# ZJU-FAST-Lab/Dftpav

Measured on AMD Instinct MI355X. Metric: trajectory solves/sec (batched), 16-piece MINCO, higher is better.
Workload: dtype f64

## Files before the change

dftpav_amd/csrc/capi.cpp:

```cpp
#include <hip/hip_runtime.h>
#include <dlfcn.h>
#include <atomic>
#include <mutex>

#include <climits>
#include <cmath>
#include <cstdio>
#include <algorithm>
#include <cstdlib>
#include <cstring>
#include <string>
#include <vector>

#include "../../include/dftpav_hip.h"
#include "device_types.h"
#include "e4_plan.h"
#include "traj_math.h"
#include "cr_trig.h"
#include "rs_math.h"
#include "search_args.h"
#include "plan_args.h"

namespace dftpav {
hipError_t launch_solver(const DevBatch &D, const DevBatch *d_dev, int mode, int threads, int grid, SchedArgs sched,
// ... 79 lines not shown
  void *d_search_ws = nullptr;
  size_t search_ws_bytes = 0;
};

struct dftpav_batch {
  dftpav_handle *h = nullptr;
  int B = 0;
  int n_active = 0;
  DevLayout L{};
  DevParams P{};
  int threads = 0;
  bool op_in_lds = false, cor_in_lds = false;
  bool have_corridor = false;
  bool sched = false;
  int slots = 0, slice = 0, hand_over = 0;
  int threads2 = 0;
  bool op_in_lds2 = false, cor_in_lds2 = false;
  int *d_queue = nullptr, *d_stragglers = nullptr, *d_stragglers2 = nullptr, *d_sflag = nullptr, *d_iota = nullptr;
  int qcap = 0;
  bool pending = false;
  unsigned *d_qctl = nullptr;
  double *d_state = nullptr;
  DevBatch *d_dev2 = nullptr;
  E4Sizes e4{}, e4b{};
  int *d_e4[2][5] = {{nullptr, nullptr, nullptr, nullptr, nullptr}, {nullptr, nullptr, nullptr, nullptr, nullptr}};
  int NptsPad = 0;
  std::vector<double> x0_host;
  bool uploaded = false;
  double t_now = 0.0, epis = 0.0;
  double *d_x0 = nullptr, *d_iniS = nullptr, *d_finS = nullptr, *d_corridor = nullptr;
  int16_t *d_pt_piece = nullptr, *d_pt_j = nullptr;
  double *d_opM[kMaxSeg] = {nullptr}, *d_opMT[kMaxSeg] = {nullptr};
  double *d_histS = nullptr, *d_histY = nullptr, *d_histU = nullptr, *d_histV = nullptr, *d_histR = nullptr;
  double *d_x_in = nullptr, *d_x_out = nullptr, *d_f = nullptr, *d_g = nullptr;
  int *d_status = nullptr, *d_success = nullptr, *d_iters = nullptr, *d_evals = nullptr;
  long long *d_hist = nullptr, *d_ticks = nullptr, *d_prof = nullptr;
  unsigned char *d_records = nullptr;
  unsigned char *h_records = nullptr;
  DevBatch *d_dev = nullptr;
  int dev_version = -1;
  DevBatch *h_stage = nullptr;
  hipEvent_t stage_ev = nullptr;
  bool stage_busy = false;
  bool prof_on = false;
  double *d_coef = nullptr, *d_dt = nullptr;
  double *d_f_eval = nullptr;
  double *d_trace = nullptr;
  double *d_cor_raw = nullptr;
  int order = DFTPAV_ORDER_DEVICE;
  int ref_S = 0;
  double *d_ref_tab = nullptr, *d_ref_scratch = nullptr;
  RefPlan ref_plan{};
  double *d_cor_t = nullptr;
  bool cor_t_dirty = true;
  bool cor_rect = false, cor_t_rect = false;
  int *d_rect_flag = nullptr;
  bool coef_override = false;
  int residency = -1;
  struct PlanCycle {
    double *d_poses = nullptr, *d_t = nullptr, *d_v = nullptr, *d_rd = nullptr;
    int *d_col = nullptr, *d_first = nullptr, *d_valid = nullptr;
    size_t n_poses = 0, n_t = 0, n_v = 0, n_rd = 0;
    std::vector<double> poses, tt, vv;
    int n_samples = 0;
    bool in_flight = false;
  } pc;
// ... 864 lines not shown
  P.surround_clearance = p.surround_clearance;
  P.max_vel[0] = p.max_forward_vel; P.max_vel[1] = p.max_backward_vel;
  P.max_acc[0] = p.max_forward_acc; P.max_acc[1] = p.max_backward_acc;
  P.max_cur[0] = p.max_forward_cur; P.max_cur[1] = p.max_backward_cur;
  P.non_sinv = p.non_sinv;
  P.mini_T = p.mini_T;
  P.fail_cost = p.fail_cost;
  double W = p.veh_width + 2 * p.half_margin, Lh = p.veh_length + 2 * p.half_margin, dcr = p.veh_d_cr;
  P.veh_length_infl = Lh;
  double le[4][2] = {{dcr + Lh / 2.0, W / 2.0}, {dcr + Lh / 2.0, -W / 2.0}, {dcr - Lh / 2.0, -W / 2.0},
                     {dcr - Lh / 2.0, W / 2.0}};
  for (int k = 0; k < 4; k++) { P.vec_le[k][0] = le[k][0]; P.vec_le[k][1] = le[k][1]; }
  P.vec_le[4][0] = le[0][0]; P.vec_le[4][1] = le[0][1];
  fill_footprint_edges(P);
  P.gear_opt = p.gear_opt;
  P.mem_size = p.lbfgs_mem_size;
  P.past = p.lbfgs_past;
  P.max_iterations = p.lbfgs_max_iterations;
  P.max_linesearch = p.lbfgs_max_linesearch;
  P.delta = p.lbfgs_delta;
  P.g_epsilon = p.lbfgs_g_epsilon;
  P.min_step = p.lbfgs_min_step;
  P.max_step = p.lbfgs_max_step;
  P.f_dec_coeff = p.lbfgs_f_dec_coeff;
  P.s_curv_coeff = p.lbfgs_s_curv_coeff;
  P.cautious_factor = p.lbfgs_cautious_factor;
  P.machine_prec = p.lbfgs_machine_prec;
}

extern "C" void dftpav_batch_destroy(dftpav_batch *b) {
  if (!b) return;
  (void)hipSetDevice(b->h->device);
  (void)hipStreamSynchronize(b->h->stream);
  void *ptrs[] = {b->d_x0, b->d_iniS, b->d_finS, b->d_corridor, b->d_pt_piece, b->d_pt_j, b->d_histS, b->d_histU, b->d_histV, b->d_histR,
                  b->d_x_in, b->d_x_out, b->d_f, b->d_g, b->d_status, b->d_success, b->d_iters, b->d_evals,
                  b->d_hist, b->d_ticks, b->d_prof, b->d_dev, b->d_coef, b->d_dt, b->d_records,
                  b->d_queue, b->d_stragglers, b->d_stragglers2, b->d_sflag, b->d_iota, b->d_qctl, b->d_state, b->d_dev2,
                  b->d_f_eval, b->d_trace, b->d_cor_raw, b->d_ref_tab, b->d_ref_scratch, b->d_cor_t, b->d_rect_flag, b->pc.d_poses, b->pc.d_t, b->pc.d_v, b->pc.d_rd, b->pc.d_col, b->pc.d_first,
                  b->pc.d_valid};
  {
    auto &v = b->h->batches;
    v.erase(std::remove(v.begin(), v.end(), b), v.end());
  }
  for (void *p : ptrs)
    if (p) (void)hipFree(p);
  if (b->h_records) (void)hipHostFree(b->h_records);
  for (int w = 0; w < 2; w++)
    for (int t = 0; t < 5; t++)
      if (b->d_e4[w][t]) (void)hipFree(b->d_e4[w][t]);
  for (int i = 0; i < kMaxSeg; i++) {
    if (b->d_opM[i]) (void)hipFree(b->d_opM[i]);
    if (b->d_opMT[i]) (void)hipFree(b->d_opMT[i]);
  }
  if (b->h_stage) (void)hipHostFree(b->h_stage);
  if (b->stage_ev) (void)hipEventDestroy(b->stage_ev);
  if (b->ev0) (void)hipEventDestroy(b->ev0);
  if (b->ev1) (void)hipEventDestroy(b->ev1);
  delete b;
}

static void fill_dev_layout(const dftpav_layout &layout, int K, int Kd, DevLayout &L) {
  L = DevLayout{};
  L.M = layout.M;
  L.H = layout.H;
  L.K = K;
  L.Kd = Kd;
  L.Kmax = L.K > L.Kd ? L.K : L.Kd;
// ... 398 lines not shown
  D.e4_groups = b->e4.groups;
  D.e4_left = b->e4.left;
  D.e4_lcap = b->e4.lcap;
  D.e4_gtab = b->d_e4[0][0];
  D.e4_ltab = b->d_e4[0][1];
  D.e4_wave = b->d_e4[0][2];
  D.e4_round = b->d_e4[0][3];
  D.e4_piece = b->d_e4[0][4];
  int off = 0;
  for (int i = 0; i < kMaxSeg; i++) {
    D.opM[i] = b->d_opM[i];
    D.opMT[i] = b->d_opMT[i];
    D.op_off[i] = off;
    if (i < b->L.M) off += 6 * b->L.piece_nums[i] * (b->L.piece_nums[i] + 5);
  }
  dftpav_handle *h = b->h;
  D.sur.S = h->S;
  D.sur_np = h->sur_pieces;
  D.sur_coef_lds = sur_coef_in_lds(b, b->threads, b->op_in_lds, b->cor_in_lds);
  D.sur.piece_off = h->d_sur_off;
  D.sur.durations = h->d_sur_dur;
  D.sur.theta = h->d_sur_theta;
  D.sur.bbox = h->d_sur_bbox;
  D.sur.coeffs = h->d_sur_coef;
  D.sur.total = h->d_sur_total;
  D.sur.start = h->d_sur_start;
  D.t_now = b->t_now;
  D.epis = b->epis;
  D.histS = b->d_histS;
  D.histY = b->d_histY;
  D.histU = b->d_histU;
  D.histV = b->d_histV;
  D.histR = b->d_histR;
  D.queue = b->d_queue;
  D.qctl = b->d_qctl;
  D.stragglers = b->d_stragglers;
  D.stragglers2 = b->d_stragglers2;
  D.qcap = b->qcap;
  D.state = b->d_state;
  D.sflag = b->d_sflag;
  D.state_stride = solver_state_doubles(b->L, b->P);
  D.x_in = b->d_x_in;
  D.x_out = b->d_x_out;
  D.f_out = b->d_f;
  D.g_out = b->d_g;
  D.f_eval = b->d_f_eval;
  D.status = b->d_status;
  D.success = b->d_success;
  D.iters = b->d_iters;
  D.evals = b->d_evals;
  D.hist_sum = b->d_hist;
  D.ticks = b->d_ticks;
  D.records = b->d_records;
  D.records_host = b->h_records;
  D.prof = b->prof_on ? b->d_prof : nullptr;
  D.coef_out = b->d_coef;
  D.dt_out = b->d_dt;
  D.trace = b->d_trace;
  D.trace_b = b->trace_b;
  D.trace_cap = b->trace_cap;
  D.trace_n = b->trace_n;
  return D;
}

static int sync_dev(dftpav_batch *b, DevBatch &D) {
  dftpav_handle *h = b->h;
// ... 257 lines not shown
  if (order == DFTPAV_ORDER_REFERENCE && b->d_trace) {
    h->err = "reference order: dftpav_batch_trace is a device-order facility -- switch the trace off first";
    return DFTPAV_E_UNSUPPORTED;
  }
  HIPCHK(h, hipSetDevice(h->device));
  if (int rc = finish_pending(b)) return rc;
  HIPCHK(h, hipStreamSynchronize(h->stream));
  if (order == DFTPAV_ORDER_REFERENCE) {
    if (!reference_order_supported(b->L, b->P, h->S)) {
      h->err = "reference order: n <= 256 variables, H <= 12 half-planes, 5 H + S + 4 <= 64 terms per point, every gear segment >= 2 pieces, 159 KB of LDS";
      return DFTPAV_E_UNSUPPORTED;
    }
    int n_cu = 256;
    hipDeviceProp_t prop;
    if (hipGetDeviceProperties(&prop, h->device) == hipSuccess && prop.multiProcessorCount > 0) n_cu = prop.multiProcessorCount;
    const RefPlan pl = reference_order_plan(b->L, b->P, h->S, b->B, n_cu, b->residency == 2, ref_options_from_env());
    if (pl.kind != kRefTeam && ensure_ring_buffers(b) != hipSuccess) {
      h->err = "reference order: no device memory for the ring of this batch";
      return DFTPAV_E_HIP;
    }
    const bool new_tab = !b->d_ref_tab || !b->d_ref_scratch || b->ref_S != h->S;
    std::vector<double> tab;
    for (int sg = 0; new_tab && sg < b->L.M; sg++) {
      std::vector<double> one;
      if (!reference_order_tables(b->L.piece_nums[sg], one)) {
        h->err = "reference order: the LU factors of this band system do not have the pattern the kernel assumes";
        return DFTPAV_E_UNSUPPORTED;
      }
      std::vector<double> packed(reference_order_table_doubles(b->L.piece_nums[sg]));
      reference_order_pack_tables(b->L.piece_nums[sg], one.data(), packed.data());
      tab.insert(tab.end(), packed.begin(), packed.end());
    }
    double *cor_t = b->d_cor_t, *d_tab = nullptr, *d_scr = nullptr;
    auto undo = [&](const char *msg) {
      if (cor_t != b->d_cor_t) (void)hipFree(cor_t);
      if (d_tab) (void)hipFree(d_tab);
      if (d_scr) (void)hipFree(d_scr);
      (void)hipGetLastError();
      h->err = msg;
      return DFTPAV_E_HIP;
    };
    if (pl.kind >= kRefQuad && !cor_t && hipMalloc(&cor_t, sizeof(double) * reference_order_quad_corridor_doubles(b->L, b->B)) != hipSuccess)
      return undo("reference order: no device memory for the QUAD shape's copy of the corridor");
    if (new_tab && (hipMalloc(&d_tab, sizeof(double) * tab.size()) != hipSuccess ||
                    hipMalloc(&d_scr, sizeof(double) * reference_order_scratch_doubles(b->L, b->B, h->S)) != hipSuccess ||
                    hipMemcpy(d_tab, tab.data(), sizeof(double) * tab.size(), hipMemcpyHostToDevice) != hipSuccess))
      return undo("reference order: no device memory for the term records of this batch");
    if (new_tab) {
      if (b->d_ref_tab) (void)hipFree(b->d_ref_tab);
      if (b->d_ref_scratch) (void)hipFree(b->d_ref_scratch);
      b->d_ref_tab = d_tab;
      b->d_ref_scratch = d_scr;
      b->ref_S = h->S;
    }
    if (pl.kind >= kRefQuad) b->cor_t_dirty = true;
    b->d_cor_t = cor_t;
    b->ref_plan = pl;
  }
  b->order = order;
  b->solved = false;
  return DFTPAV_OK;
}
extern "C" int dftpav_batch_get_order(const dftpav_batch *b) { return b ? b->order : DFTPAV_E_INVALID; }

extern "C" int dftpav_batch_eval(dftpav_batch *b, const double *x, double *f, double *g) {
  if (!b || !x || !b->uploaded || !b->have_corridor) return DFTPAV_E_INVALID;
  dftpav_handle *h = b->h;
  const size_t nb = (size_t)b->B * b->L.n;
  HIPCHK(h, hipSetDevice(h->device));
  HIPCHK(h, hipMemcpyAsync(b->d_x_in, x, sizeof(double) * nb, hipMemcpyHostToDevice, h->stream));
  DevBatch D;
  if (int rc = sync_dev(b, D)) return rc;
  HIPCHK(h, launch_for(b, D, kModeEval));
  if (f) HIPCHK(h, hipMemcpyAsync(f, b->d_f_eval, sizeof(double) * b->B, hipMemcpyDeviceToHost, h->stream));
  if (g) HIPCHK(h, hipMemcpyAsync(g, b->d_g, sizeof(double) * nb, hipMemcpyDeviceToHost, h->stream));
  HIPCHK(h, hipStreamSynchronize(h->stream));
  return DFTPAV_OK;
}

static int launch_stragglers(dftpav_batch *b, const DevBatch &D, int source) {
  dftpav_handle *h = b->h;
  DevBatch D2 = D;
  D2.op_in_lds = b->op_in_lds2 ? 1 : 0;
  D2.cor_in_lds = b->cor_in_lds2 ? 1 : 0;
  D2.sur_coef_lds = sur_coef_in_lds(b, b->threads2, b->op_in_lds2, b->cor_in_lds2);
  D2.e4_rounds = b->e4b.rounds;
  D2.e4_groups = b->e4b.groups;
  D2.e4_left = b->e4b.left;
  D2.e4_lcap = b->e4b.lcap;
// ... 1715 lines not shown
```

dftpav_amd/csrc/device_types.h:

```cpp
#pragma once
#include <cstdint>

#ifndef DFTPAV_HD
#if defined(__HIPCC__)
#define DFTPAV_HD __host__ __device__
#else
#define DFTPAV_HD
#endif
#endif

namespace dftpav {

constexpr int kMaxSeg = 8;
constexpr int kWave = 64;
constexpr int kMaxThreads = 1024;

struct DevParams {
  double wei_obs, wei_surround, wei_feas, wei_time;
  double surround_clearance;
  double max_vel[2], max_acc[2], max_cur[2];
  double non_sinv, mini_T, fail_cost;
  double veh_length_infl;
  double vec_le[5][2];
  double edge_d[4][2], edge_len[4], edge_rlen[4];
// ... 42 lines not shown
};

inline int e4_group_size(int points) { return points >= 32 ? 32 : (points >= 16 ? 16 : 0); }

struct DevBatch {
  DevLayout L;
  DevParams P;
  int B;
  const double *x0;
  const double *iniS;
  const double *finS;
  const double *corridor;
  int NptsPad;
  const int16_t *pt_piece;
  const int16_t *pt_j;
  const double *opM[kMaxSeg];
  const double *opMT[kMaxSeg];
  int op_in_lds;
  int cor_in_lds;
  int e4_rounds, e4_groups, e4_left, e4_lcap;
  const int *e4_gtab;
  const int *e4_ltab;
  const int *e4_wave;
  const int *e4_round;
  const int *e4_piece;
  int op_off[kMaxSeg];
  DevSurround sur;
  int sur_np;
  int sur_coef_lds;
  double t_now, epis;
  double *histS, *histY;
  double *histU, *histV;
  double *histR;
  int *queue;
  unsigned *qctl;
  int *stragglers;
  int *stragglers2;
  int qcap;
  double *state;
  int *sflag;
  int state_stride;
  const double *x_in;
  double *x_out;
  double *f_out;
  double *g_out;
  double *f_eval;
  int *status, *success, *iters, *evals;
  long long *hist_sum;
  unsigned char *records;
  unsigned char *records_host;
  long long *ticks;
  long long *prof;
  double *coef_out;
  double *dt_out;
  double *trace;
  int trace_b, trace_cap, trace_n;
};

enum KernelMode { kModeSolve = 0, kModeEval = 1, kModeCoeffs = 2 };

constexpr int kAltTag = 1 << 30;
struct SchedArgs {
  int source;
  int slice;
  int hand_over;
  const DevBatch *alt;
};
inline int solver_state_doubles(const DevLayout &L, const DevParams &P) { (void)P; return 5 * L.npad + 24 + 8; }

struct RefOptions {
  int shape;
  int waves;
  int threads;
  int quad_waves;
  int quad_hand;
  int slice;
  int slots;
  bool exact_div;
  bool verbose;
};

enum RefKind { kRefTeam = 0, kRefWave = 1, kRefQuad = 3, kRefQuadSeg = 5 };
struct RefShape {
  int kind;
  int threads;
  int wg_per_cu;
  int slots;
  int slice;
  int slots_wide;
  int hand;
// ... 26 lines not shown
```

dftpav_amd/csrc/solver_ref4.hip:

```cpp
#include <hip/hip_runtime.h>
#include <cstdio>
#include <cstdlib>
#include <algorithm>

#include "ref_order_common.h"
#include "quad_common.h"

namespace dftpav {
namespace reford {

constexpr int kQLcap = 7;
#ifndef DFTPAV_Q4_WAVES_PER_EU
#define DFTPAV_Q4_WAVES_PER_EU 1
#endif
constexpr int kQ4WavesPerCU = 4 * DFTPAV_Q4_WAVES_PER_EU;

struct Q4 {
  ldsd_t xs, gs;
  ldsd_t bnd;
  ldsd_t tw;
  ldsd_t st;
  ldsd_t alpha;
  ldsd_t tl;
  ldsi_t ist;
// ... 594 lines not shown
  const bool e0 = l < n, e1 = 16 + l < n;
  v.xp0 = e0 ? q.xs[l] : 0.0;
  v.xp1 = e1 ? q.xs[16 + l] : 0.0;
  v.gp0 = e0 ? q.gs[l] : 0.0;
  v.gp1 = e1 ? q.gs[16 + l] : 0.0;
  const double dginit = row_sum32(v.gp0 * v.d0, v.gp1 * v.d1, n, l);
  const double step = q.st[sSTEP];
  if (!(step > 0.0)) {
    if (l == 0) q.ist[iRET] = -1006;
    return false;
  }
  if (0.0 < dginit) {
    if (l == 0) q.ist[iRET] = -1005;
    return false;
  }
  if (l == 0) {
    q.st[sFINIT] = q.st[sFX];
    q.st[sDGINIT] = dginit;
    q.st[sDGTEST] = P.f_dec_coeff * dginit;
    q.st[sDSTEST] = P.s_curv_coeff * dginit;
    q.st[sMU] = 0.0;
    q.st[sNU] = P.max_step;
    q.st[sSTP] = step;
    q.ist[iCOUNT] = 0;
    q.ist[iBRACKT] = 0;
    q.ist[iTOUCHED] = 0;
  }
  if (e0) q.xs[l] = v.xp0 + step * v.d0;
  if (e1) q.xs[16 + l] = v.xp1 + step * v.d1;
  return true;
}

constexpr int kQB = 8;
struct QBlk {
  d2_t a[kQB], b[kQB];
  d2_t yr[kQB];
};
typedef double __attribute__((ext_vector_type(2))) qd2_t;
template <int DIR>
__device__ __forceinline__ void q4_load_blk(QBlk &R, gcd2_t hS, gcd2_t hR, int npad, int m, int la, int lb, int &jl) {
#pragma unroll
  for (int u = 0; u < kQB; u++) {
    const gcd2_t row = hS + (size_t)jl * npad + la;
    R.a[u] = row[0];
    R.b[u] = row[16];
    R.yr[u] = hR[jl];
    if (DIR < 0) jl = jl == 0 ? m - 1 : jl - 1;
    else jl = jl == m - 1 ? 0 : jl + 1;
  }
}
__device__ __forceinline__ void q4_pin_blk(QBlk &R) {
#pragma unroll
  for (int u = 0; u < kQB; u++)
    asm volatile("" : "+v"(R.a[u].x), "+v"(R.a[u].y), "+v"(R.b[u].x), "+v"(R.b[u].y), "+v"(R.yr[u].x), "+v"(R.yr[u].y));
}
template <bool EXACT>
__device__ __forceinline__ void q4_first_steps(const QBlk &R, const Q4 &q, int i0, int bound, int m, int n, int l, bool exact, int &j, double &d0, double &d1) {
#pragma unroll
  for (int u = 0; u < kQB; u++) {
    if (i0 + u < bound) {
      j = j == 0 ? m - 1 : j - 1;
      const double dot = row_sum32(R.a[u].x * d0, R.b[u].x * d1, n, l);
      const double a = EXACT && exact ? dot / R.yr[u].x : div_by_rcp<false>(dot, R.yr[u].x, R.yr[u].y);
      if (l == 0) q.alpha[j] = a;
      const double na = -a;
      d0 = d0 + na * R.a[u].y;
      d1 = d1 + na * R.b[u].y;
    }
  }
}
template <bool EXACT>
__device__ __forceinline__ void q4_second_steps(const QBlk &R, const Q4 &q, int i0, int bound, int m, int n, int l, bool exact, int &j, double &d0, double &d1) {
#pragma unroll
  for (int u = 0; u < kQB; u++) {
    if (i0 + u < bound) {
      const double al = q.alpha[j];
      const double dot = row_sum32(R.a[u].y * d0, R.b[u].y * d1, n, l);
      const double beta = EXACT && exact ? dot / R.yr[u].x : div_by_rcp<false>(dot, R.yr[u].x, R.yr[u].y);
      const double cf = al - beta;
      d0 = d0 + cf * R.a[u].x;
      d1 = d1 + cf * R.b[u].x;
      j = j == m - 1 ? 0 : j + 1;
    }
  }
}
template <bool EXACT>
__device__ __forceinline__ void q4_two_loop(const Q4 &q, gcd2_t hS, gcd2_t hR, int npad, int m, int n, int l, int bound, int ne, bool exact, double sc0, double &d0,
                                            double &d1) {
  const int la = l, lb = 16 + l;
  QBlk A, B;
  int j = ne;
  int jl = ne == 0 ? m - 1 : ne - 1;
  q4_load_blk<-1>(A, hS, hR, npad, m, la, lb, jl);
#pragma unroll 1
  for (int i0 = 0; i0 < bound; i0 += 2 * kQB) {
    q4_pin_blk(A);
    q4_load_blk<-1>(B, hS, hR, npad, m, la, lb, jl);
    q4_first_steps<EXACT>(A, q, i0, bound, m, n, l, exact, j, d0, d1);
    q4_pin_blk(B);
    q4_load_blk<-1>(A, hS, hR, npad, m, la, lb, jl);
    q4_first_steps<EXACT>(B, q, i0 + kQB, bound, m, n, l, exact, j, d0, d1);
  }
  d0 = d0 * sc0;
  d1 = d1 * sc0;
  __builtin_amdgcn_fence(__ATOMIC_SEQ_CST, "wavefront");
  jl = j;
  q4_load_blk<+1>(A, hS, hR, npad, m, la, lb, jl);
#pragma unroll 1
  for (int i0 = 0; i0 < bound; i0 += 2 * kQB) {
    q4_pin_blk(A);
    q4_load_blk<+1>(B, hS, hR, npad, m, la, lb, jl);
    q4_second_steps<EXACT>(A, q, i0, bound, m, n, l, exact, j, d0, d1);
    q4_pin_blk(B);
    q4_load_blk<+1>(A, hS, hR, npad, m, la, lb, jl);
    q4_second_steps<EXACT>(B, q, i0 + kQB, bound, m, n, l, exact, j, d0, d1);
  }
}

__device__ __forceinline__ void q4_advance(const DevBatch &D, const Q4 &q, QVec &v, double f, gd_t hS, gd_t hR, int l, Prof &pr) {
  const DevParams &P = D.P;
  const int n = D.L.n, m = P.mem_size, npad = D.L.npad;
  const bool e0 = l < n, e1 = 16 + l < n;
  int action = kActEval;
  if (q.ist[iPHASE] == 0) {
    const double g0 = e0 ? q.gs[l] : 0.0, g1 = e1 ? q.gs[16 + l] : 0.0;
    const double x0 = e0 ? q.xs[l] : 0.0, x1 = e1 ? q.xs[16 + l] : 0.0;
    v.d0 = e0 ? -g0 : 0.0;
    v.d1 = e1 ? -g1 : 0.0;
    const double gmax = row_max16(fmax(fabs(g0), fabs(g1))), xmax = row_max16(fmax(fabs(x0), fabs(x1)));
    const double dd = row_sum32((-g0) * (-g0), (-g1) * (-g1), n, l);
    __builtin_amdgcn_fence(__ATOMIC_SEQ_CST, "wavefront");
    if (l == 0) {
      q.st[sFX] = f;
      q.st[sPF0] = f;
      q.ist[iEVALS] = 1;
      q.ist[iEND] = 0;
      q.ist[iBOUND] = 0;
      q.ist[iHISTLO] = 0;
      q.ist[iHISTHI] = 0;
      q.ist[iPHASE] = 1;
    }
    if (gmax / fmax(1.0, xmax) < P.g_epsilon) {
      if (l == 0) {
        q.ist[iRET] = 0;
        q.ist[iK] = 0;
      }
      action = kActDone;
    } else {
      if (l == 0) {
        q.st[sSTEP] = 1.0 / sqrt(dd);
        q.ist[iK] = 1;
      }
      __threadfence_block();
      if (!q4_begin_iteration(P, q, v, n, l)) action = kActDone;
// ... 109 lines not shown
      if (0 < P.past) {
        const int slot = k % P.past;
        const double pf = q.st[sPF0 + slot];
        __threadfence_block();
        if (P.past <= k) {
          const double rate = fabs(pf - fx) / fmax(1.0, fabs(fx));
          if (rate < P.delta) ret = 1;
        }
        if (ret == kGoOn && l == 0) q.st[sPF0 + slot] = fx;
      }
      if (ret == kGoOn && P.max_iterations != 0 && P.max_iterations <= k) ret = -1008;
    }
    if (ret != kGoOn) {
      if (l == 0) {
        q.ist[iRET] = ret;
        q.ist[iACTION] = kActDone;
      }
      return;
    }
  }
  ++k;
  pr.tick(6);
  const int end = q.ist[iEND];
  int bound = q.ist[iBOUND];
  __threadfence_block();
  if (l == 0) q.ist[iK] = k;

  const double sv0 = e0 ? x0 - v.xp0 : 0.0, sv1 = e1 ? x1 - v.xp1 : 0.0;
  const double yv0 = e0 ? g0 - v.gp0 : 0.0, yv1 = e1 ? g1 - v.gp1 : 0.0;
  if (e0) {
    d2_t sy;
    sy.x = sv0;
    sy.y = yv0;
    ((gd2_t)hS)[(size_t)end * npad + l] = sy;
  }
  if (e1) {
    d2_t sy;
    sy.x = sv1;
    sy.y = yv1;
    ((gd2_t)hS)[(size_t)end * npad + 16 + l] = sy;
  }
  v.d0 = e0 ? -g0 : 0.0;
  v.d1 = e1 ? -g1 : 0.0;
  const double ys = row_sum32(yv0 * sv0, yv1 * sv1, n, l);
  const double yy = row_sum32(yv0 * yv0, yv1 * yv1, n, l);
  const double ss = row_sum32(sv0 * sv0, sv1 * sv1, n, l);
  const double gpgp = row_sum32(v.gp0 * v.gp0, v.gp1 * v.gp1, n, l);
  if (l == 0) {
    d2_t yr;
    yr.x = ys;
    yr.y = 1.0 / ys;
    ((gd2_t)hR)[end] = yr;
    if (!rcp_route_ok(ys)) q.ist[iSLOWDIV] = 1;
  }
  const double cau = ss * sqrt(gpgp) * P.cautious_factor;
  pr.tick(7);
  if (ys > cau) {
    ++bound;
    bound = m < bound ? m : bound;
    const int ne = end + 1 == m ? 0 : end + 1;
    __threadfence_block();
    const bool exact = q.ist[iSLOWDIV] != 0;
    double d0 = v.d0, d1 = v.d1;
    if (__builtin_amdgcn_ballot_w64(exact) != 0ull) q4_two_loop<true>(q, (gcd2_t)hS, (gcd2_t)hR, npad, m, n, l, bound, ne, exact, ys / yy, d0, d1);
    else q4_two_loop<false>(q, (gcd2_t)hS, (gcd2_t)hR, npad, m, n, l, bound, ne, exact, ys / yy, d0, d1);
    v.d0 = e0 ? d0 : 0.0;
    v.d1 = e1 ? d1 : 0.0;
    if (l == 0) {
      q.ist[iEND] = ne;
      q.ist[iBOUND] = bound;
      long long hs = ((long long)q.ist[iHISTHI] << 32) | (unsigned int)q.ist[iHISTLO];
      hs += bound;
      q.ist[iHISTLO] = (int)(hs & 0xffffffffLL);
      q.ist[iHISTHI] = (int)(hs >> 32);
    }
  }
  if (l == 0) q.st[sSTEP] = 1.0;
  pr.tick(8);
  __threadfence_block();
  const bool ok = q4_begin_iteration(P, q, v, n, l);
  if (l == 0) q.ist[iACTION] = ok ? kActEval : kActDone;
  pr.tick(6);
}

__device__ inline void q4_state_io(const DevBatch &D, const Q4 &q, QVec &v, int b, int l, bool save) {
  const int n = D.L.n, npad = D.L.npad;
  double *rec = D.state + (size_t)b * D.state_stride;
  for (int h = 0; h < 2; h++) {
    const int e = 16 * h + l;
    if (e >= n) {
      if (!save) {
        q.xs[e] = 0.0;
        q.gs[e] = 0.0;
        if (h == 0) { v.xp0 = 0.0; v.gp0 = 0.0; v.d0 = 0.0; } else { v.xp1 = 0.0; v.gp1 = 0.0; v.d1 = 0.0; }
      }
      continue;
    }
    if (save) {
// ... 75 lines not shown
        act = true;
        resumed = ring && D.sflag[b] == 1;
        if (resumed) {
          q4_state_io(D, q, v, b, l, false);
        } else {
          const double *xsrc = (mode == kModeSolve) ? D.x0 : D.x_in;
          for (int h = 0; h < 2; h++) {
            const int e = 16 * h + l;
            q.xs[e] = e < n ? xsrc[(size_t)b * n + e] : 0.0;
            q.gs[e] = 0.0;
          }
          v = QVec{0.0, 0.0, 0.0, 0.0, 0.0, 0.0};
          q.ist[l] = (l == iSLOWDIV && force_exact_div) ? 1 : 0;
        }
        if (l < 12) q.bnd[l] = l < 6 ? D.iniS[(size_t)b * 6 + l] : D.finS[(size_t)b * 6 + (l - 6)];
        tick0 = wall_clock64();
        pr.start(D.prof != nullptr && mode == kModeSolve && l == 0, D.prof + (size_t)b * 12, resumed);
        __builtin_amdgcn_fence(__ATOMIC_SEQ_CST, "wavefront");
      }
    }
    if (__builtin_amdgcn_ballot_w64(act) == 0ull) break;
    if (act) {
      const gcd_t cor = RECT ? (gcd_t)(cor_t + ((size_t)b * JP * 80 + l) * 2) : (gcd_t)(cor_t + (size_t)b * L.H * 4 * cpitch + l);
      const gd_t ovf = (gd_t)(scratch + (size_t)b * scratch_per_traj);
      const double f = q4_eval<FAST, RECT>(D, q, dl, tab, cor, cpitch, ovf, l, pr);
      if (mode == kModeEval) {
        for (int h = 0; h < 2; h++) {
          const int e = 16 * h + l;
          if (e < n) D.g_out[(size_t)b * n + e] = q.gs[e];
        }
        if (l == 0) D.f_eval[b] = f;
        act = false;
      } else {
        const gd_t hS = (gd_t)(D.histS + (size_t)b * mem * L.npad * 2);
        const gd_t hR = (gd_t)(D.histR + (size_t)b * mem * 2);
        q4_advance(D, q, v, f, hS, hR, l, pr);
        __builtin_amdgcn_fence(__ATOMIC_SEQ_CST, "wavefront");
        if (q.ist[iACTION] == kActDone) {
          for (int h = 0; h < 2; h++) {
            const int e = 16 * h + l;
            if (e < n) D.x_out[(size_t)b * n + e] = q.xs[e];
          }
          if (l == 0) {
            const double fx = q.st[sFX];
            const int ret = q.ist[iRET];
            D.f_out[b] = fx;
            D.status[b] = ret;
            D.iters[b] = q.ist[iK];
            D.evals[b] = q.ist[iEVALS];
            D.hist_sum[b] = ((long long)q.ist[iHISTHI] << 32) | (unsigned int)q.ist[iHISTLO];
            {
              double *rec = reinterpret_cast<double *>(D.records + (size_t)16 * b);
              rec[0] = fx;
              int *ri = reinterpret_cast<int *>(rec + 1);
              ri[0] = ret;
              ri[1] = q.ist[iK];
            }
            if (D.records_host != nullptr) {
              double *rh = reinterpret_cast<double *>(D.records_host + (size_t)16 * b);
              rh[0] = fx;
              int *rj = reinterpret_cast<int *>(rh + 1);
              rj[0] = ret;
              rj[1] = q.ist[iK];
            }
            D.ticks[b] = (resumed ? D.ticks[b] : 0) + (wall_clock64() - tick0);
            int ok = (ret == 0 || ret == 1 || ret == 2 || ret == -1008 || ret == -1009) ? 1 : 0;
            if (fx >= D.P.fail_cost) ok = 0;
            D.success[b] = ok;
            if (ring) {
// ... 60 lines not shown
    const bool nan = (C & ~sign) > 0x7ff0000000000000ull || (S & ~sign) > 0x7ff0000000000000ull;
    const bool ok = !nan && n[0][0] == (S ^ sign) && n[0][1] == C && n[2][0] == S && n[2][1] == (C ^ sign) && n[3][0] == (C ^ sign) && n[3][1] == (S ^ sign);
    if (!ok) *flag = 1;
  }
}

__global__ void q4_corridor_rect_kernel(const double *__restrict__ cor, d2_t *__restrict__ out, int B, int NptsPad, int N, int K, int Kd, int JP) {
  const size_t total = (size_t)B * JP * 80;
  for (size_t i = (size_t)blockIdx.x * blockDim.x + threadIdx.x; i < total; i += (size_t)gridDim.x * blockDim.x) {
    const int p = (int)(i & 15);
    const int u = (int)((i >> 4) % 5);
    const size_t r = i / 80;
    const int j = (int)(r % JP);
    const size_t b = r / JP;
    d2_t v = {0.0, 0.0};
    if (p < N) {
      const int Kp = (p == 0 || p == N - 1) ? Kd : K;
      const int pt0 = p == 0 ? 0 : (Kd + 1) + (p - 1) * (K + 1);
      if (j <= Kp) {
        const int c0 = u == 0 ? 4 : 4 * (u - 1) + 2;
        const double *src = cor + (b * 16 + c0) * NptsPad + pt0 + j;
        v.x = src[0];
        v.y = src[NptsPad];
      }
    }
    out[i] = v;
  }
}

}

bool reference_order_quad_supported(const DevLayout &L, const DevParams &P, int S) {
  if (L.M != 1 || S != 0 || L.n > 32 || L.Ntot > 16 || L.Ntot < 2 || L.H < 1 || L.H > 5) return false;
  return reford::q4_shared_bytes(L.Ntot) + 4 * reford::q4_team_bytes(P.mem_size) + reford::q4_dense_bytes() <= 160 * 1024;
}
size_t reference_order_quad_corridor_doubles(const DevLayout &L, int B) { return (size_t)B * L.H * 4 * (L.Kmax + 1) * 16; }
QuadSizes reference_order_quad_sizes(const DevLayout &L, const DevParams &P) {
  return {reford::q4_shared_bytes(L.Ntot), reford::q4_team_bytes(P.mem_size) + (reford::q4_dense_bytes() + 3) / 4, reford::kQ4WavesPerCU, 768};
}
hipError_t launch_quad_corridor(const DevBatch &D, double *cor_t, bool rect, hipStream_t stream) {
  const DevLayout &L = D.L;
  const size_t total = rect ? (size_t)D.B * (L.Kmax + 1) * 80 : reference_order_quad_corridor_doubles(L, D.B);
  const int grid = (int)std::min<size_t>((total + 255) / 256, 65536);
  if (rect)
    hipLaunchKernelGGL(reford::q4_corridor_rect_kernel, dim3(grid), dim3(256), 0, stream, D.corridor, reinterpret_cast<reford::d2_t *>(cor_t), D.B, D.NptsPad, L.Ntot, L.K,
                       L.Kd, L.Kmax + 1);
  else
    hipLaunchKernelGGL(reford::q4_corridor_kernel, dim3(grid), dim3(256), 0, stream, D.corridor, cor_t, D.B, L.H * 4, D.NptsPad, L.Ntot, L.K, L.Kd, L.Kmax + 1);
  return hipGetLastError();
}
hipError_t launch_quad_rect_check(const double *corridor, int B, int Npts, int NptsPad, int *d_flag, hipStream_t stream) {
  hipError_t e = hipMemsetAsync(d_flag, 0, sizeof(int), stream);
  if (e != hipSuccess) return e;
  const size_t total = (size_t)B * Npts;
  const int grid = (int)std::min<size_t>((total + 255) / 256, 65536);
  hipLaunchKernelGGL(reford::q4_rect_check_kernel, dim3(grid), dim3(256), 0, stream, corridor, B, Npts, NptsPad, d_flag);
  return hipGetLastError();
}
QuadKernel ref4_kernel_for(bool fast, bool rect) {
  if (fast && rect) return &reford::ref4_kernel<true, true>;
  return fast ? &reford::ref4_kernel<true, false> : &reford::ref4_kernel<false, false>;
}

}
```

Measured before the change: 38940.

## Mirror L-BFGS history ring ends to remove per-row wrap checks in quad two-loop

```diff
diff --git a/dftpav_amd/csrc/capi.cpp b/dftpav_amd/csrc/capi.cpp
--- a/dftpav_amd/csrc/capi.cpp
+++ b/dftpav_amd/csrc/capi.cpp
@@ -135,6 +135,7 @@
   int16_t *d_pt_piece = nullptr, *d_pt_j = nullptr;
   double *d_opM[kMaxSeg] = {nullptr}, *d_opMT[kMaxSeg] = {nullptr};
   double *d_histS = nullptr, *d_histY = nullptr, *d_histU = nullptr, *d_histV = nullptr, *d_histR = nullptr;
+  double *d_histM = nullptr;
   double *d_x_in = nullptr, *d_x_out = nullptr, *d_f = nullptr, *d_g = nullptr;
   int *d_status = nullptr, *d_success = nullptr, *d_iters = nullptr, *d_evals = nullptr;
   long long *d_hist = nullptr, *d_ticks = nullptr, *d_prof = nullptr;
@@ -1065,7 +1066,7 @@
   if (!b) return;
   (void)hipSetDevice(b->h->device);
   (void)hipStreamSynchronize(b->h->stream);
-  void *ptrs[] = {b->d_x0, b->d_iniS, b->d_finS, b->d_corridor, b->d_pt_piece, b->d_pt_j, b->d_histS, b->d_histU, b->d_histV, b->d_histR,
+  void *ptrs[] = {b->d_x0, b->d_iniS, b->d_finS, b->d_corridor, b->d_pt_piece, b->d_pt_j, b->d_histS, b->d_histU, b->d_histV, b->d_histR, b->d_histM,
                   b->d_x_in, b->d_x_out, b->d_f, b->d_g, b->d_status, b->d_success, b->d_iters, b->d_evals,
                   b->d_hist, b->d_ticks, b->d_prof, b->d_dev, b->d_coef, b->d_dt, b->d_records,
                   b->d_queue, b->d_stragglers, b->d_stragglers2, b->d_sflag, b->d_iota, b->d_qctl, b->d_state, b->d_dev2,
@@ -1530,6 +1531,7 @@
   D.histU = b->d_histU;
   D.histV = b->d_histV;
   D.histR = b->d_histR;
+  D.histM = b->d_histM;
   D.queue = b->d_queue;
   D.qctl = b->d_qctl;
   D.stragglers = b->d_stragglers;
@@ -1853,8 +1855,10 @@
       tab.insert(tab.end(), packed.begin(), packed.end());
     }
     double *cor_t = b->d_cor_t, *d_tab = nullptr, *d_scr = nullptr;
+    double *hist_m = b->d_histM;
     auto undo = [&](const char *msg) {
       if (cor_t != b->d_cor_t) (void)hipFree(cor_t);
+      if (hist_m != b->d_histM) (void)hipFree(hist_m);
       if (d_tab) (void)hipFree(d_tab);
       if (d_scr) (void)hipFree(d_scr);
       (void)hipGetLastError();
@@ -1863,6 +1867,10 @@
     };
     if (pl.kind >= kRefQuad && !cor_t && hipMalloc(&cor_t, sizeof(double) * reference_order_quad_corridor_doubles(b->L, b->B)) != hipSuccess)
       return undo("reference order: no device memory for the QUAD shape's copy of the corridor");
+    if (pl.kind == kRefQuad && !hist_m &&
+        (hipMalloc(&hist_m, sizeof(double) * quad_mirror_doubles(b->L, b->B)) != hipSuccess ||
+         hipMemset(hist_m, 0, sizeof(double) * quad_mirror_doubles(b->L, b->B)) != hipSuccess))
+      return undo("reference order: no device memory for the QUAD shape's mirror of the history ends");
     if (new_tab && (hipMalloc(&d_tab, sizeof(double) * tab.size()) != hipSuccess ||
                     hipMalloc(&d_scr, sizeof(double) * reference_order_scratch_doubles(b->L, b->B, h->S)) != hipSuccess ||
                     hipMemcpy(d_tab, tab.data(), sizeof(double) * tab.size(), hipMemcpyHostToDevice) != hipSuccess))
@@ -1876,6 +1884,8 @@
     }
     if (pl.kind >= kRefQuad) b->cor_t_dirty = true;
     b->d_cor_t = cor_t;
+    b->d_histM = hist_m;
+    b->dev_version = -1;
     b->ref_plan = pl;
   }
   b->order = order;
diff --git a/dftpav_amd/csrc/device_types.h b/dftpav_amd/csrc/device_types.h
--- a/dftpav_amd/csrc/device_types.h
+++ b/dftpav_amd/csrc/device_types.h
@@ -98,6 +98,7 @@
   double *histS, *histY;
   double *histU, *histV;
   double *histR;
+  double *histM;
   int *queue;
   unsigned *qctl;
   int *stragglers;
@@ -122,6 +123,9 @@
   double *trace;
   int trace_b, trace_cap, trace_n;
 };
+
+constexpr int kQuadMirrorRows = 16;
+inline size_t quad_mirror_doubles(const DevLayout &L, int B) { return (size_t)B * kQuadMirrorRows * L.npad * 2; }
 
 enum KernelMode { kModeSolve = 0, kModeEval = 1, kModeCoeffs = 2 };
 
diff --git a/dftpav_amd/csrc/solver_ref4.hip b/dftpav_amd/csrc/solver_ref4.hip
--- a/dftpav_amd/csrc/solver_ref4.hip
+++ b/dftpav_amd/csrc/solver_ref4.hip
@@ -650,94 +650,141 @@
 }
 
 constexpr int kQB = 8;
-struct QBlk {
+constexpr int kQNpad = 64;
+static_assert(kQuadMirrorRows == 2 * kQB, "DevBatch::histM holds kQB rows of either end of a ring");
+template <bool Y3> struct QBlk {
   d2_t a[kQB], b[kQB];
-  d2_t yr[kQB];
+  d2_t yr[Y3 ? kQB : 1];
 };
 typedef double __attribute__((ext_vector_type(2))) qd2_t;
-template <int DIR>
-__device__ __forceinline__ void q4_load_blk(QBlk &R, gcd2_t hS, gcd2_t hR, int npad, int m, int la, int lb, int &jl) {
+
+#define DFTPAV_FMAC_BCAST15 \
+  DFTPAV_FMAC_BCAST(0) DFTPAV_FMAC_BCAST(1) DFTPAV_FMAC_BCAST(2) DFTPAV_FMAC_BCAST(3) DFTPAV_FMAC_BCAST(4) DFTPAV_FMAC_BCAST(5) DFTPAV_FMAC_BCAST(6) \
+  DFTPAV_FMAC_BCAST(7) DFTPAV_FMAC_BCAST(8) DFTPAV_FMAC_BCAST(9) DFTPAV_FMAC_BCAST(10) DFTPAV_FMAC_BCAST(11) DFTPAV_FMAC_BCAST(12) \
+  DFTPAV_FMAC_BCAST(13) DFTPAV_FMAC_BCAST(14)
+__device__ __forceinline__ double row_chain15(double acc, double v) {
+  const double one = 1.0;
+  asm volatile("s_nop 1\n\t" DFTPAV_FMAC_BCAST15 : "+v"(acc) : "v"(v), "v"(one));
+  return acc;
+}
+template <bool Y3> __device__ __forceinline__ double q4_rec_sum(double p0, double p1, int n) {
+  double acc = row_chain16(0.0, p0);
+  if (n > 16) acc = Y3 ? row_chain16(acc, p1) : row_chain15(acc, p1);
+  return acc;
+}
+
+template <int DIR, bool Y3>
+__device__ __forceinline__ void q4_load_blk(QBlk<Y3> &R, gcd2_t hS, gcd2_t hM, gcd2_t hR, int m, int l, int &jl) {
+  const bool wrap = DIR < 0 ? jl < kQB - 1 : jl > m - kQB;
+  const int mr = DIR < 0 ? kQB + jl : jl - (m - kQB);
+  const gcd2_t row = (wrap ? hM + mr * kQNpad : hS + jl * kQNpad) + l;
 #pragma unroll
   for (int u = 0; u < kQB; u++) {
-    const gcd2_t row = hS + (size_t)jl * npad + la;
-    R.a[u] = row[0];
-    R.b[u] = row[16];
-    R.yr[u] = hR[jl];
-    if (DIR < 0) jl = jl == 0 ? m - 1 : jl - 1;
-    else jl = jl == m - 1 ? 0 : jl + 1;
-  }
-}
-__device__ __forceinline__ void q4_pin_blk(QBlk &R) {
-#pragma unroll
-  for (int u = 0; u < kQB; u++)
-    asm volatile("" : "+v"(R.a[u].x), "+v"(R.a[u].y), "+v"(R.b[u].x), "+v"(R.b[u].y), "+v"(R.yr[u].x), "+v"(R.yr[u].y));
-}
-template <bool EXACT>
-__device__ __forceinline__ void q4_first_steps(const QBlk &R, const Q4 &q, int i0, int bound, int m, int n, int l, bool exact, int &j, double &d0, double &d1) {
+    R.a[u] = row[DIR * u * kQNpad];
+    R.b[u] = row[DIR * u * kQNpad + 16];
+  }
+  if (Y3) {
+    int jr = jl;
+#pragma unroll
+    for (int u = 0; u < kQB; u++) {
+      R.yr[Y3 ? u : 0] = hR[jr];
+      if (DIR < 0) jr = jr == 0 ? m - 1 : jr - 1;
+      else jr = jr == m - 1 ? 0 : jr + 1;
+    }
+  }
+  if (DIR < 0) {
+    jl -= kQB;
+    jl = jl < 0 ? jl + m : jl;
+  } else {
+    jl += kQB;
+    jl = jl >= m ? jl - m : jl;
+  }
+}
+template <bool Y3> __device__ __forceinline__ void q4_pin_blk(QBlk<Y3> &R) {
+#pragma unroll
+  for (int u = 0; u < kQB; u++) {
+    asm volatile("" : "+v"(R.a[u].x), "+v"(R.a[u].y), "+v"(R.b[u].x), "+v"(R.b[u].y));
+    if (Y3) asm volatile("" : "+v"(R.yr[Y3 ? u : 0].x), "+v"(R.yr[Y3 ? u : 0].y));
+  }
+}
+template <bool Y3> __device__ __forceinline__ d2_t q4_blk_yr(const QBlk<Y3> &R, int u) {
+  if (Y3) return R.yr[Y3 ? u : 0];
+  d2_t yr;
+  yr.x = mov_dpp<0x15F>(R.b[u].x);
+  yr.y = mov_dpp<0x15F>(R.b[u].y);
+  return yr;
+}
+template <bool EXACT, bool Y3>
+__device__ __forceinline__ void q4_first_steps(const QBlk<Y3> &R, ldsd_t al, int i0, int bound, int n, int l, bool exact, double &d0, double &d1) {
 #pragma unroll
   for (int u = 0; u < kQB; u++) {
     if (i0 + u < bound) {
-      j = j == 0 ? m - 1 : j - 1;
-      const double dot = row_sum32(R.a[u].x * d0, R.b[u].x * d1, n, l);
-      const double a = EXACT && exact ? dot / R.yr[u].x : div_by_rcp<false>(dot, R.yr[u].x, R.yr[u].y);
-      if (l == 0) q.alpha[j] = a;
+      const d2_t yr = q4_blk_yr<Y3>(R, u);
+      const double dot = q4_rec_sum<Y3>(R.a[u].x * d0, R.b[u].x * d1, n);
+      const double a = EXACT && exact ? dot / yr.x : div_by_rcp<false>(dot, yr.x, yr.y);
+      if (l == 0) al[u] = a;
       const double na = -a;
       d0 = d0 + na * R.a[u].y;
       d1 = d1 + na * R.b[u].y;
     }
   }
 }
-template <bool EXACT>
-__device__ __forceinline__ void q4_second_steps(const QBlk &R, const Q4 &q, int i0, int bound, int m, int n, int l, bool exact, int &j, double &d0, double &d1) {
+template <bool EXACT, bool Y3>
+__device__ __forceinline__ void q4_second_steps(const QBlk<Y3> &R, ldscd_t al, int i0, int bound, int n, int l, bool exact, double &d0, double &d1) {
 #pragma unroll
   for (int u = 0; u < kQB; u++) {
     if (i0 + u < bound) {
-      const double al = q.alpha[j];
-      const double dot = row_sum32(R.a[u].y * d0, R.b[u].y * d1, n, l);
-      const double beta = EXACT && exact ? dot / R.yr[u].x : div_by_rcp<false>(dot, R.yr[u].x, R.yr[u].y);
-      const double cf = al - beta;
+      const double av = al[kQB - 1 - u];
+      const d2_t yr = q4_blk_yr<Y3>(R, u);
+      const double dot = q4_rec_sum<Y3>(R.a[u].y * d0, R.b[u].y * d1, n);
+      const double beta = EXACT && exact ? dot / yr.x : div_by_rcp<false>(dot, yr.x, yr.y);
+      const double cf = av - beta;
       d0 = d0 + cf * R.a[u].x;
       d1 = d1 + cf * R.b[u].x;
-      j = j == m - 1 ? 0 : j + 1;
-    }
-  }
-}
-template <bool EXACT>
-__device__ __forceinline__ void q4_two_loop(const Q4 &q, gcd2_t hS, gcd2_t hR, int npad, int m, int n, int l, int bound, int ne, bool exact, double sc0, double &d0,
+    }
+  }
+}
+template <bool EXACT, bool Y3>
+__device__ __forceinline__ void q4_two_loop(const Q4 &q, gcd2_t hS, gcd2_t hM, gcd2_t hR, int m, int n, int l, int bound, int ne, bool exact, double sc0, double &d0,
                                             double &d1) {
-  const int la = l, lb = 16 + l;
-  QBlk A, B;
-  int j = ne;
+  QBlk<Y3> A, B;
   int jl = ne == 0 ? m - 1 : ne - 1;
-  q4_load_blk<-1>(A, hS, hR, npad, m, la, lb, jl);
+  q4_load_blk<-1>(A, hS, hM, hR, m, l, jl);
 #pragma unroll 1
   for (int i0 = 0; i0 < bound; i0 += 2 * kQB) {
     q4_pin_blk(A);
-    q4_load_blk<-1>(B, hS, hR, npad, m, la, lb, jl);
-    q4_first_steps<EXACT>(A, q, i0, bound, m, n, l, exact, j, d0, d1);
+    q4_load_blk<-1>(B, hS, hM, hR, m, l, jl);
+    q4_first_steps<EXACT>(A, q.alpha + i0, i0, bound, n, l, exact, d0, d1);
     q4_pin_blk(B);
-    q4_load_blk<-1>(A, hS, hR, npad, m, la, lb, jl);
-    q4_first_steps<EXACT>(B, q, i0 + kQB, bound, m, n, l, exact, j, d0, d1);
+    q4_load_blk<-1>(A, hS, hM, hR, m, l, jl);
+    q4_first_steps<EXACT>(B, q.alpha + (i0 + kQB), i0 + kQB, bound, n, l, exact, d0, d1);
   }
   d0 = d0 * sc0;
   d1 = d1 * sc0;
   __builtin_amdgcn_fence(__ATOMIC_SEQ_CST, "wavefront");
-  jl = j;
-  q4_load_blk<+1>(A, hS, hR, npad, m, la, lb, jl);
+  jl = ne - bound;
+  jl = jl < 0 ? jl + m : jl;
+  q4_load_blk<+1>(A, hS, hM, hR, m, l, jl);
 #pragma unroll 1
   for (int i0 = 0; i0 < bound; i0 += 2 * kQB) {
+    const ldscd_t al = (ldscd_t)(q.alpha + (bound - kQB - i0));
     q4_pin_blk(A);
-    q4_load_blk<+1>(B, hS, hR, npad, m, la, lb, jl);
-    q4_second_steps<EXACT>(A, q, i0, bound, m, n, l, exact, j, d0, d1);
+    q4_load_blk<+1>(B, hS, hM, hR, m, l, jl);
+    q4_second_steps<EXACT>(A, al, i0, bound, n, l, exact, d0, d1);
     q4_pin_blk(B);
-    q4_load_blk<+1>(A, hS, hR, npad, m, la, lb, jl);
-    q4_second_steps<EXACT>(B, q, i0 + kQB, bound, m, n, l, exact, j, d0, d1);
-  }
-}
-
-__device__ __forceinline__ void q4_advance(const DevBatch &D, const Q4 &q, QVec &v, double f, gd_t hS, gd_t hR, int l, Prof &pr) {
+    q4_load_blk<+1>(A, hS, hM, hR, m, l, jl);
+    q4_second_steps<EXACT>(B, al - kQB, i0 + kQB, bound, n, l, exact, d0, d1);
+  }
+}
+__device__ __forceinline__ void q4_store_pair(gd_t hS, gd_t hM, int m, int end, int e, d2_t v) {
+  ((gd2_t)hS)[(size_t)end * kQNpad + e] = v;
+  if (end < kQB) ((gd2_t)hM)[(kQB + end) * kQNpad + e] = v;
+  if (end >= m - kQB) ((gd2_t)hM)[(end - (m - kQB)) * kQNpad + e] = v;
+}
+
+__device__ __forceinline__ void q4_advance(const DevBatch &D, const Q4 &q, QVec &v, double f, gd_t hS, gd_t hM, gd_t hR, int l, Prof &pr) {
   const DevParams &P = D.P;
-  const int n = D.L.n, m = P.mem_size, npad = D.L.npad;
+  const int n = D.L.n, m = P.mem_size;
   const bool e0 = l < n, e1 = 16 + l < n;
   int action = kActEval;
   if (q.ist[iPHASE] == 0) {
@@ -913,13 +960,13 @@
     d2_t sy;
     sy.x = sv0;
     sy.y = yv0;
-    ((gd2_t)hS)[(size_t)end * npad + l] = sy;
+    q4_store_pair(hS, hM, m, end, l, sy);
   }
   if (e1) {
     d2_t sy;
     sy.x = sv1;
     sy.y = yv1;
-    ((gd2_t)hS)[(size_t)end * npad + 16 + l] = sy;
+    q4_store_pair(hS, hM, m, end, 16 + l, sy);
   }
   v.d0 = e0 ? -g0 : 0.0;
   v.d1 = e1 ? -g1 : 0.0;
@@ -934,6 +981,13 @@
     ((gd2_t)hR)[end] = yr;
     if (!rcp_route_ok(ys)) q.ist[iSLOWDIV] = 1;
   }
+  const bool y3 = n > 31;
+  if (l == 15 && !y3) {
+    d2_t yr;
+    yr.x = ys;
+    yr.y = 1.0 / ys;
+    q4_store_pair(hS, hM, m, end, 31, yr);
+  }
   const double cau = ss * sqrt(gpgp) * P.cautious_factor;
   pr.tick(7);
   if (ys > cau) {
@@ -943,8 +997,14 @@
     __threadfence_block();
     const bool exact = q.ist[iSLOWDIV] != 0;
     double d0 = v.d0, d1 = v.d1;
-    if (__builtin_amdgcn_ballot_w64(exact) != 0ull) q4_two_loop<true>(q, (gcd2_t)hS, (gcd2_t)hR, npad, m, n, l, bound, ne, exact, ys / yy, d0, d1);
-    else q4_two_loop<false>(q, (gcd2_t)hS, (gcd2_t)hR, npad, m, n, l, bound, ne, exact, ys / yy, d0, d1);
+    const gcd2_t cS = (gcd2_t)hS, cM = (gcd2_t)hM, cR = (gcd2_t)hR;
+    if (__builtin_amdgcn_ballot_w64(exact) != 0ull) {
+      if (y3) q4_two_loop<true, true>(q, cS, cM, cR, m, n, l, bound, ne, exact, ys / yy, d0, d1);
+      else q4_two_loop<true, false>(q, cS, cM, cR, m, n, l, bound, ne, exact, ys / yy, d0, d1);
+    } else {
+      if (y3) q4_two_loop<false, true>(q, cS, cM, cR, m, n, l, bound, ne, exact, ys / yy, d0, d1);
+      else q4_two_loop<false, false>(q, cS, cM, cR, m, n, l, bound, ne, exact, ys / yy, d0, d1);
+    }
     v.d0 = e0 ? d0 : 0.0;
     v.d1 = e1 ? d1 : 0.0;
     if (l == 0) {
@@ -1086,9 +1146,10 @@
         if (l == 0) D.f_eval[b] = f;
         act = false;
       } else {
-        const gd_t hS = (gd_t)(D.histS + (size_t)b * mem * L.npad * 2);
+        const gd_t hS = (gd_t)(D.histS + (size_t)b * mem * kQNpad * 2);
+        const gd_t hM = (gd_t)(D.histM + (size_t)b * kQuadMirrorRows * kQNpad * 2);
         const gd_t hR = (gd_t)(D.histR + (size_t)b * mem * 2);
-        q4_advance(D, q, v, f, hS, hR, l, pr);
+        q4_advance(D, q, v, f, hS, hM, hR, l, pr);
         __builtin_amdgcn_fence(__ATOMIC_SEQ_CST, "wavefront");
         if (q.ist[iACTION] == kActDone) {
           for (int h = 0; h < 2; h++) {
@@ -1215,6 +1276,7 @@
 
 bool reference_order_quad_supported(const DevLayout &L, const DevParams &P, int S) {
   if (L.M != 1 || S != 0 || L.n > 32 || L.Ntot > 16 || L.Ntot < 2 || L.H < 1 || L.H > 5) return false;
+  if (L.npad != reford::kQNpad || P.mem_size < reford::kQB) return false;
   return reford::q4_shared_bytes(L.Ntot) + 4 * reford::q4_team_bytes(P.mem_size) + reford::q4_dense_bytes() <= 160 * 1024;
 }
 size_t reference_order_quad_corridor_doubles(const DevLayout &L, int B) { return (size_t)B * L.H * 4 * (L.Kmax + 1) * 16; }
```

New measurement: 42720, median of 6. 1.1x the previous value.
